# facebookresearch/video-long-term-feature-banks

Hardware: AMD Instinct MI355X
Metric: clips/sec fwd+bwd R50-I3D-NL+LFB-NL, 32x224^2 synthetic (higher is better)
Workload: dtype mix; 1 GPU; ava_r50_lfb_nl fwd+bwd+allreduce+sgd, 8 clips/GPU (global batch 8), RoIs/clip ~ U{1..5} (33 on rank 0), 32x224x224 clips; parallelism=dp1

## Files before the change

video-long-term-feature-banks_amd/csrc/vlfb_gemm_nt.h:

```cpp
#pragma once
#include "vlfb_gemm_common.h"

namespace vlfb {
namespace {

template <typename T, typename OutT, int BM, int BN, bool IDENT, bool DGRAD, bool PACKW, int RB, bool PRE, int NW,
          int ST = 2, bool UT = false, bool PAIR = false, bool W2I = false>
__global__ __launch_bounds__(64 * NW) void gemm_nt_kernel(const GP p) {
  static_assert(!W2I || (sizeof(T) == 2 && RB == 128 && ST == 2 && UT && DGRAD && !PAIR), "W2I: 16-bit unit-stride DGRAD on the tap cursor");
  static_assert(!PAIR || (sizeof(T) == 2 && RB == 128 && ST == 2 && (IDENT || UT) && !PACKW && !DGRAD), "PAIR: fp16 planes, plain rows or UT FPROP");
  static_assert(!UT || (!IDENT && !PACKW), "UT is for gathered, unpacked operands");
  constexpr int NTHR = 64 * NW;
  constexpr int NWN = NW / 2;
  constexpr int EPC = Elem<T>::EPC;
  constexpr int CPRW = RB / 16;
  constexpr int RPPS = NTHR / CPRW;
  constexpr int A_IT = BM / RPPS, B_IT = BN / RPPS;
  constexpr int WM = BM / 2, WN = BN / NWN;
  constexpr int FM = WM / 16, FN = WN / 16;
  constexpr int BUF = (BM + BN) * RB;
  constexpr int KSTEPS = sizeof(T) == 4 ? 1 : RB / 64;
  extern __shared__ __attribute__((aligned(16))) char smem[];

  const int tid = threadIdx.x, lane = tid & 63, wave = tid >> 6;
  const int wm = wave / NWN, wn = wave % NWN;
  const int l15 = lane & 15, g = lane >> 4;

  const int nwg = p.tiles_m * p.tiles_n;
  const int bid = xcd_remap(blockIdx.x, nwg);
  const int tile_m = bid / p.tiles_n, tile_n = bid - tile_m * p.tiles_n;
  int m0 = tile_m * BM;
  const int n0 = tile_n * BN;
  const int z = blockIdx.z;
  constexpr bool S2C = DGRAD && !UT && !IDENT && !PACKW;
  bool s2 = false;
  int s2_ph = 0, s2_pw = 0;
  if constexpr (S2C) {
    s2 = p.s2 != 0;
    if (s2) {
      const int cls = tile_m / p.s2_tpc;
      m0 = (tile_m - cls * p.s2_tpc) * BM;
      s2_ph = cls >> 1; s2_pw = cls & 1;
    }
  }
  const int mrows = s2 ? p.s2_mq : p.M;
  auto row_coords = [&](int m) {
    if constexpr (S2C) {
      if (s2) {
        const int w2n = p.Wr >> 1, h2n = p.Hr >> 1;
        RowC r;
        const int w2 = m % w2n; int q = m / w2n;
        const int h2 = q % h2n; q /= h2n;
        r.t = q % p.Tr; r.n = q / p.Tr;
        r.h = 2 * h2 + s2_ph; r.w = 2 * w2 + s2_pw;
        return r;
      }
    }
    return decode_row(p, m);
  };
  auto row_pos = [&](int m) -> long long {
    if constexpr (S2C) {
      if (s2) {
        const RowC r = row_coords(m);
        return (long long)((r.n * p.Tr + r.t) * p.Hr + r.h) * p.Wr + r.w;
      }
    }
    return m;
  };

  const char* Ab = p.A + (long long)z * p.a_bs * (long long)sizeof(T);
  const char* Bb = p.B + (long long)z * p.b_bs * (long long)sizeof(T);

  const int cc = tid % CPRW;
  const int r0 = tid / CPRW;
  const int ccg = cc ^ swz_key<RB>(r0);
  const unsigned a_cb = PAIR ? (unsigned)(ccg & 3) * 16u + (unsigned)(ccg >> 2) * (unsigned)p.a_ps * 2u : (unsigned)(ccg * EPC) * (unsigned)sizeof(T);
  const unsigned b_cb = PAIR ? (unsigned)(ccg & 3) * 16u + (unsigned)(ccg >> 2) * (unsigned)p.b_ps * 2u : (unsigned)(ccg * EPC) * (unsigned)sizeof(T);
  const int KTB = PAIR ? RB / 2 : RB;
  const int wave_u = __builtin_amdgcn_readfirstlane(wave);

  RowC arow[A_IT];
  bool aok[A_IT];
  int upix[UT ? A_IT : 1];
#pragma unroll
  for (int i = 0; i < A_IT; ++i) {
    int m = m0 + r0 + RPPS * i;
    aok[i] = m < mrows;
    if (!IDENT) arow[i] = row_coords(aok[i] ? m : 0);
    if (UT) {
      RowC& r = arow[i];
      if (!DGRAD) { r.t = r.t * p.st - p.pt; r.h = r.h * p.sh - p.ph; r.w = r.w * p.sw - p.pw; }
      else { r.t += p.pt; r.h += p.ph; r.w += p.pw; }
      upix[i] = ((r.n * p.Ts + r.t) * p.Hs + r.h) * p.Ws + r.w;
    }
  }
  unsigned boff[B_IT], aoff[(IDENT || UT) ? A_IT : 1];
#pragma unroll
  for (int i = 0; i < B_IT; ++i) {
    const int n = n0 + r0 + RPPS * i;
    boff[i] = n < p.Ncols ? (unsigned)(n * p.ldb) * (unsigned)sizeof(T) + b_cb : kOOB;
  }
  if (IDENT || UT) {
#pragma unroll
    for (int i = 0; i < A_IT; ++i) {
      const int m = m0 + r0 + RPPS * i;
      if (IDENT) aoff[i] = aok[i] ? (unsigned)(m * p.lda) * (unsigned)sizeof(T) + a_cb : kOOB;
      else aoff[i] = (unsigned)(upix[i] * p.lda) * (unsigned)sizeof(T) + a_cb;
    }
  }
  const auto rsA = make_rsrc(Ab, p.a_bytes);
  const auto rsB = make_rsrc(Bb, p.b_bytes);
  int u_a = 0, u_b = 0, u_c = 0, u_ci = 0;

  int ktiles = (p.K * (int)sizeof(T) + (PAIR ? RB / 2 : RB) - 1) / (PAIR ? RB / 2 : RB);
  if constexpr (W2I) ktiles *= 2;
  int s2_kpt = 1, s2_b0 = 0, s2_c0 = 0, s2_nb = 0, s2_nc = 0;
  int s2_a = 0, s2_ib = 0, s2_ic = 0, s2_in = 0;
  if constexpr (S2C) {
    if (s2) {
      s2_kpt = p.Cs * (int)sizeof(T) / RB;
      s2_b0 = (s2_ph + p.ph) & 1; s2_c0 = (s2_pw + p.pw) & 1;
      s2_nb = p.kh > s2_b0 ? (p.kh - s2_b0 + 1) >> 1 : 0;
      s2_nc = p.kw > s2_c0 ? (p.kw - s2_c0 + 1) >> 1 : 0;
      ktiles = p.kt * s2_nb * s2_nc * s2_kpt;
    }
  }
  auto s2_next_kt = [&]() {
    const int tap = (s2_a * p.kh + s2_b0 + 2 * s2_ib) * p.kw + s2_c0 + 2 * s2_ic;
    const int kt = tap * s2_kpt + s2_in;
    if (++s2_in == s2_kpt) {
      s2_in = 0;
      if (++s2_ic == s2_nc) { s2_ic = 0; if (++s2_ib == s2_nb) { s2_ib = 0; ++s2_a; } }
    }
    return kt;
  };

  auto load_tile = [&](int kt_seq, int buf) {
    int kt = kt_seq;
    if constexpr (S2C) {
      if (s2) kt = s2_next_kt();
    }
    const int kc = PAIR ? kt * (CPRW / 2) + (ccg & 3) : kt * CPRW + ccg;
    TapC tap;
    if (IDENT || UT) { tap.ok = kc * EPC < p.K; tap.a = tap.b = tap.c = tap.ci = 0; }
    else tap = decode_tap<T, PACKW>(p, kc);
    const bool kok = W2I || kc * EPC < p.K;
    {
      char* xa = smem + (W2I ? (kt_seq >> 1) & 1 : buf) * BUF + wave_u * 1024;
      char* wb = smem + buf * BUF + BM * RB + wave_u * 1024;
      const unsigned kbyte = (unsigned)kt * KTB;
      if (UT) {
        const int sgn = DGRAD ? -1 : 1;
        const int da = sgn * u_a * p.dt, db = sgn * u_b * p.dh, dc = sgn * u_c * p.dw;
        const unsigned dbyte = (unsigned)(((da * p.Hs + db) * p.Ws + dc) * p.lda + u_ci) * (unsigned)sizeof(T);
        if (!W2I || !(kt_seq & 1)) {
#pragma unroll
          for (int i = 0; i < A_IT; ++i) {
            const bool ok = aok[i] && (unsigned)(arow[i].t + da) < (unsigned)p.Ts &&
                            (unsigned)(arow[i].h + db) < (unsigned)p.Hs && (unsigned)(arow[i].w + dc) < (unsigned)p.Ws;
            bufglds16(rsA, ok ? aoff[i] + dbyte : kOOB, 0, xa + i * (RPPS * RB));
          }
          u_ci += (PAIR ? RB / 2 : RB) / (int)sizeof(T);
          if (u_ci >= p.Cs) {
            u_ci = 0;
            if (++u_c == p.kw) { u_c = 0; if (++u_b == p.kh) { u_b = 0; ++u_a; } }
          }
        }
      } else if (IDENT) {
#pragma unroll
        for (int i = 0; i < A_IT; ++i) bufglds16(rsA, kok ? aoff[i] : kOOB, kbyte, xa + i * (RPPS * RB));
      } else {
#pragma unroll
        for (int i = 0; i < A_IT; ++i) {
          unsigned off;
          if (PACKW) {
            const int ts = arow[i].t * p.st - p.pt + tap.a * p.dt;
            const int hs = arow[i].h * p.sh - p.ph + tap.b * p.dh;
            const bool ok = aok[i] && tap.ok && (unsigned)ts < (unsigned)p.Ts && (unsigned)hs < (unsigned)p.Hs;
            const int w0 = arow[i].w * p.sw - p.pw + tap.c;
            const int pix = ((arow[i].n * p.Ts + ts) * p.Hs + hs) * p.Ws + w0;
            off = ok ? (unsigned)pix * 4u * (unsigned)sizeof(T) : kOOB;
          } else {
            bool ok;
            const long long e = src_offset<DGRAD>(p, arow[i], tap, ok);
            off = (ok && aok[i] && tap.ok) ? (unsigned)e * (unsigned)sizeof(T) : kOOB;
          }
          bufglds16(rsA, off, 0, xa + i * (RPPS * RB));
        }
      }
#pragma unroll
      for (int i = 0; i < B_IT; ++i) bufglds16(rsB, kok ? boff[i] : kOOB, kbyte, wb + i * (RPPS * RB));
    }
  };
  constexpr int LPT = A_IT + B_IT;
  auto ring_wait = [&](int newer) {
    if (newer >= 3 && ST >= 5) asm volatile("s_waitcnt vmcnt(%0)" ::"n"(3 * LPT) : "memory");
    else if (newer == 2 && ST >= 4) asm volatile("s_waitcnt vmcnt(%0)" ::"n"(2 * LPT) : "memory");
    else if (newer == 1 && ST >= 3) asm volatile("s_waitcnt vmcnt(%0)" ::"n"(1 * LPT) : "memory");
    else asm volatile("s_waitcnt vmcnt(0)" ::: "memory");
  };

  f32x4_v acc[FN][FM];
#pragma unroll
  for (int a = 0; a < FN; ++a)
#pragma unroll
    for (int b = 0; b < FM; ++b) acc[a][b] = f32x4_v{0.f, 0.f, 0.f, 0.f};

  char* Ob = p.O + (long long)z * p.o_bs * (long long)sizeof(OutT);
  const char* Rb = p.R ? p.R + (long long)z * p.r_bs * (long long)sizeof(T) : nullptr;
  const char* Mb = p.Mask ? p.Mask + (long long)z * p.r_bs * (long long)sizeof(T) : nullptr;
  const char* R2b = p.R2 ? p.R2 + (long long)z * p.r_bs * (long long)sizeof(T) : nullptr;
  char* O2b = p.O2 ? p.O2 + (long long)z * p.o_bs * ((PAIR || sizeof(T) == 2) ? 2ll : (long long)sizeof(OutT)) : nullptr;
  constexpr int EPT = 16 / (int)sizeof(OutT);
  constexpr int TPR = BN / EPT;
  constexpr int RPP = NTHR / TPR;
  constexpr int NPASS = BM / RPP;
  const int tc = tid % TPR, tr = tid / TPR;
  const int ncol = n0 + tc * EPT;
  constexpr bool PREM = PRE && !PAIR;
  constexpr bool PRE2 = PRE && PAIR;
  const bool nt = p.nt_epi != 0;
  uint4 rpre[PRE ? NPASS : 1], mpre[PREM ? NPASS : 1], r2pre[PRE2 ? NPASS : 1];
  if (PRE) {
#pragma unroll
    for (int gp = 0; gp < NPASS; ++gp) {
      const int m = m0 + gp * RPP + tr;
      const bool ok = m < mrows && ncol < p.Ncols;
      const long long off = (row_pos(ok ? m : 0) * p.ldr + ncol) * (long long)sizeof(T);
      rpre[gp] = ld16_epi(nt, src_or_zero(Rb ? Rb : Ab, off, ok && Rb != nullptr));
      if constexpr (PRE2) r2pre[gp] = ld16_epi(nt, src_or_zero(R2b ? R2b : Ab, off, ok && R2b != nullptr));
      if constexpr (PREM) mpre[gp] = ld16_epi(nt, src_or_zero(Mb ? Mb : Ab, off, ok && Mb != nullptr));
    }
  }
  (void)R2b; (void)O2b;

  static_assert(ST >= 2 && ST <= 5 && 3 * LPT < 64, "ring depth / vmcnt immediate");
#pragma unroll
  for (int s0 = 0; s0 < ST - 1; ++s0)
    if (s0 < ktiles) load_tile(s0, s0);

  int cur = 0, nxt = ST - 1;
  if constexpr (W2I) {
    constexpr bool HOLD = !PRE;
    for (int kt = 0; kt < ktiles; kt += 2) {
      typename Mma<T>::Frag xf[KSTEPS][FM];
      asm volatile("s_waitcnt vmcnt(0)" ::: "memory");
      asm volatile("s_barrier" ::: "memory");
      load_tile(kt + 1, 1);
      {
        const char* xa = smem + ((kt >> 1) & 1) * BUF;
        const char* wb = smem + BM * RB;
        if constexpr (HOLD) {
#pragma unroll
          for (int ks = 0; ks < KSTEPS; ++ks)
#pragma unroll
            for (int i = 0; i < FM; ++i) xf[ks][i] = Mma<T>::template load<RB>(xa, wm * WM + i * 16 + l15, ks, g);
        }
#pragma unroll
        for (int ks = 0; ks < KSTEPS; ++ks) {
          typename Mma<T>::Frag wf[FN];
          if constexpr (!HOLD) {
#pragma unroll
            for (int i = 0; i < FM; ++i) xf[ks][i] = Mma<T>::template load<RB>(xa, wm * WM + i * 16 + l15, ks, g);
          }
#pragma unroll
          for (int j = 0; j < FN; ++j) wf[j] = Mma<T>::template load<RB>(wb, wn * WN + j * 16 + l15, ks, g);
#pragma unroll
          for (int j = 0; j < FN; ++j)
#pragma unroll
            for (int i = 0; i < FM; ++i) acc[j][i] = Mma<T>::mma(wf[j], xf[ks][i], acc[j][i]);
        }
      }
      asm volatile("s_waitcnt vmcnt(0)" ::: "memory");
      asm volatile("s_barrier" ::: "memory");
      if (kt + 2 < ktiles) load_tile(kt + 2, 0);
      {
        const char* xa = smem + ((kt >> 1) & 1) * BUF;
        const char* wb = smem + BUF + BM * RB;
#pragma unroll
        for (int ks = 0; ks < KSTEPS; ++ks) {
          typename Mma<T>::Frag wf[FN];
          if constexpr (!HOLD) {
#pragma unroll
            for (int i = 0; i < FM; ++i) xf[ks][i] = Mma<T>::template load<RB>(xa, wm * WM + i * 16 + l15, ks, g);
          }
#pragma unroll
          for (int j = 0; j < FN; ++j) wf[j] = Mma<T>::template load<RB>(wb, wn * WN + j * 16 + l15, ks, g);
#pragma unroll
          for (int j = 0; j < FN; ++j)
#pragma unroll
            for (int i = 0; i < FM; ++i) acc[j][i] = Mma<T>::mma(wf[j], xf[ks][i], acc[j][i]);
        }
      }
    }
  } else
  for (int kt = 0; kt < ktiles; ++kt) {
    const int ahead = ktiles - 1 - kt;
    ring_wait(ahead < ST - 2 ? ahead : ST - 2);
    asm volatile("s_barrier" ::: "memory");
    const bool more = kt + ST - 1 < ktiles;
    if (more) load_tile(kt + ST - 1, nxt);
    const char* xa = smem + cur * BUF;
    const char* wb = xa + BM * RB;
    if constexpr (PAIR) {
      typename Mma<T>::Frag xh[FM], xl[FM], wh[FN], wl[FN];
#pragma unroll
      for (int i = 0; i < FM; ++i) {
        xh[i] = Mma<T>::template load<RB>(xa, wm * WM + i * 16 + l15, 0, g);
        xl[i] = Mma<T>::template load<RB>(xa, wm * WM + i * 16 + l15, 1, g);
      }
#pragma unroll
      for (int j = 0; j < FN; ++j) {
        wh[j] = Mma<T>::template load<RB>(wb, wn * WN + j * 16 + l15, 0, g);
        wl[j] = Mma<T>::template load<RB>(wb, wn * WN + j * 16 + l15, 1, g);
      }
#pragma unroll
      for (int j = 0; j < FN; ++j)
#pragma unroll
        for (int i = 0; i < FM; ++i) acc[j][i] = Mma<T>::mma(wl[j], xh[i], acc[j][i]);
#pragma unroll
      for (int j = 0; j < FN; ++j)
#pragma unroll
        for (int i = 0; i < FM; ++i) acc[j][i] = Mma<T>::mma(wh[j], xl[i], acc[j][i]);
#pragma unroll
      for (int j = 0; j < FN; ++j)
#pragma unroll
        for (int i = 0; i < FM; ++i) acc[j][i] = Mma<T>::mma(wh[j], xh[i], acc[j][i]);
    } else {
#pragma unroll
    for (int ks = 0; ks < KSTEPS; ++ks) {
      typename Mma<T>::Frag xf[FM], wf[FN];
#pragma unroll
      for (int i = 0; i < FM; ++i) xf[i] = Mma<T>::template load<RB>(xa, wm * WM + i * 16 + l15, ks, g);
#pragma unroll
      for (int j = 0; j < FN; ++j) wf[j] = Mma<T>::template load<RB>(wb, wn * WN + j * 16 + l15, ks, g);
#pragma unroll
      for (int j = 0; j < FN; ++j)
#pragma unroll
        for (int i = 0; i < FM; ++i) acc[j][i] = Mma<T>::mma(wf[j], xf[i], acc[j][i]);
    }
    }
    cur = cur + 1 == ST ? 0 : cur + 1;
    nxt = nxt + 1 == ST ? 0 : nxt + 1;
  }
  __syncthreads();

  if (p.vec_epi) {
    constexpr int CPR = BN / 4;
    const int epi = p.epi;
    auto stage = [&](int h) {
      if (epi == 1 || wm == h) {
#pragma unroll
        for (int i = 0; i < FM; ++i) {
          const int row = (epi == 1 ? wm * WM : 0) + i * 16 + l15;
#pragma unroll
          for (int j = 0; j < FN; ++j) {
            const int c = (wn * WN + j * 16 + g * 4) >> 2;
            *reinterpret_cast<float4*>(smem + ((row * CPR + (c ^ (row & 7))) << 4)) =
                make_float4(acc[j][i][0] * p.alpha, acc[j][i][1] * p.alpha, acc[j][i][2] * p.alpha,
                            acc[j][i][3] * p.alpha);
          }
        }
      }
    };
    stage(0);
    __syncthreads();
#pragma unroll
    for (int gp = 0; gp < NPASS; ++gp) {
      if (gp == NPASS / 2 && epi == 2) {
        __syncthreads();
        stage(1);
        __syncthreads();
      }
      const int trow = gp * RPP + tr;
      const int row = (epi == 2 && gp >= NPASS / 2) ? trow - BM / 2 : trow;
      const int m = m0 + trow;
      if (m < mrows && ncol < p.Ncols) {
        const long long mpos = row_pos(m);
        float v[EPT];
#pragma unroll
        for (int q = 0; q < EPT / 4; ++q) {
          const int c = tc * (EPT / 4) + q;
          const float4 t = *reinterpret_cast<const float4*>(smem + ((row * CPR + (c ^ (row & 7))) << 4));
          v[4 * q] = t.x; v[4 * q + 1] = t.y; v[4 * q + 2] = t.z; v[4 * q + 3] = t.w;
        }
        if (p.bias_mode == VLFB_BIAS_COL) {
#pragma unroll
          for (int e = 0; e < EPT; ++e) v[e] += p.bias[ncol + e];
        } else if (p.bias_mode == VLFB_BIAS_ROW) {
          const float b = p.bias[m];
#pragma unroll
          for (int e = 0; e < EPT; ++e) v[e] += b;
        }
        const long long ridx = mpos * p.ldr + ncol;
        if (Rb) {
          float r[EPT];
          if (PRE) unpack_elems<T, EPT>(rpre[PRE ? gp : 0], r);
          else load_elems_epi<T, EPT>(nt, reinterpret_cast<const T*>(Rb) + ridx, r);
#pragma unroll
          for (int e = 0; e < EPT; ++e) v[e] += r[e];
        }
        if constexpr (sizeof(T) == 2 && sizeof(OutT) == 2) {
          if (R2b) {
            float r[EPT];
            if constexpr (PRE2) unpack_elems<T, EPT>(r2pre[PRE2 ? gp : 0], r);
            else load_elems_epi<T, EPT>(nt, reinterpret_cast<const T*>(R2b) + ridx, r);
#pragma unroll
            for (int e = 0; e < EPT; ++e) v[e] += r[e];
          }
        }
        if (p.relu) {
#pragma unroll
          for (int e = 0; e < EPT; ++e) v[e] = fmaxf(v[e], 0.f);
        }
        if (Mb && !PAIR) {
          float r[EPT];
          if (PREM) unpack_elems<T, EPT>(mpre[PREM ? gp : 0], r);
          else load_elems_epi<T, EPT>(nt, reinterpret_cast<const T*>(Mb) + ridx, r);
#pragma unroll
          for (int e = 0; e < EPT; ++e) v[e] = r[e] > 0.f ? v[e] : 0.f;
        }
        OutT* o = reinterpret_cast<OutT*>(Ob) + mpos * p.ldo + ncol;
        if (sizeof(OutT) == 4) {
          st16_epi(nt, o, make_float4(v[0], v[1], v[2], v[3]));
          if constexpr (PAIR) {
            if (O2b) st8_epi(nt, reinterpret_cast<unsigned short*>(O2b) + mpos * p.ldo + ncol,
                             make_uint2(pack_h2_pos(v[0], v[1]), pack_h2_pos(v[2 % EPT], v[3 % EPT])));
          } else if constexpr (sizeof(T) == 2) {
            if (O2b) st8_epi(nt, reinterpret_cast<T*>(O2b) + mpos * p.ldo + ncol,
                             make_uint2(Elem<T>::pack2(v[0], v[1]), Elem<T>::pack2(v[2 % EPT], v[3 % EPT])));
          }
        } else {
          const uint4 hv = make_uint4(Elem<OutT>::pack2(v[0], v[1]), Elem<OutT>::pack2(v[2 % EPT], v[3 % EPT]),
                                      Elem<OutT>::pack2(v[4 % EPT], v[5 % EPT]), Elem<OutT>::pack2(v[6 % EPT], v[7 % EPT]));
          st16_epi(nt, o, hv);
          if (O2b) {
            float h[EPT];
            unpack_elems<OutT, EPT>(hv, h);
            st16_epi(nt, reinterpret_cast<OutT*>(O2b) + mpos * p.ldo + ncol,
                     make_uint4(Elem<OutT>::pack2(v[0] - h[0], v[1] - h[1]), Elem<OutT>::pack2(v[2 % EPT] - h[2 % EPT], v[3 % EPT] - h[3 % EPT]),
                                Elem<OutT>::pack2(v[4 % EPT] - h[4 % EPT], v[5 % EPT] - h[5 % EPT]), Elem<OutT>::pack2(v[6 % EPT] - h[6 % EPT], v[7 % EPT] - h[7 % EPT])));
          }
        }
      }
    }
    return;
  }
  const bool vec_ok = (p.ldo & 3) == 0;
#pragma unroll
  for (int i = 0; i < FM; ++i) {
    const int m = m0 + wm * WM + i * 16 + l15;
    if (m >= mrows) continue;
    const long long mpos = row_pos(m);
#pragma unroll
    for (int j = 0; j < FN; ++j) {
      const int nb = n0 + wn * WN + j * 16 + g * 4;
      if (nb >= p.Ncols) continue;
      const int cnt = (p.Ncols - nb) < 4 ? (p.Ncols - nb) : 4;
      float v[4];
#pragma unroll
      for (int r = 0; r < 4; ++r) {
        float x = acc[j][i][r] * p.alpha;
        if (r < cnt) {
          if (p.bias_mode == VLFB_BIAS_COL) x += p.bias[nb + r];
          else if (p.bias_mode == VLFB_BIAS_ROW) x += p.bias[m];
          if (Rb) x += ld_elem<T>(Rb, mpos * p.ldr + nb + r);
          if (p.relu) x = fmaxf(x, 0.f);
          if (Mb) x = ld_elem<T>(Mb, mpos * p.ldr + nb + r) > 0.f ? x : 0.f;
        }
        v[r] = x;
      }
      store4<OutT>(Ob, mpos * p.ldo + nb, v, cnt, vec_ok);
    }
  }
}

}
}
```

video-long-term-feature-banks_amd/csrc/vlfb_gemm_pair.hip:

```cpp
#include "vlfb_gemm_nt.h"
#include "vlfb_gemm_nt8.h"

namespace vlfb {
namespace {

template <typename K>
void launch_pair_k(K kernel, dim3 grid, int threads, size_t lds, const GP& gp, hipStream_t s) {
  static bool configured = false;
  if (!configured) {
    (void)hipFuncSetAttribute(reinterpret_cast<const void*>(kernel), hipFuncAttributeMaxDynamicSharedMemorySize, 80 * 1024);
    configured = true;
  }
  hipLaunchKernelGGL(kernel, grid, dim3(threads), lds, s, gp);
}

template <typename OutT, int BN, bool PRE>
void launch_pair_shape(const GP& gp, bool ident, dim3 grid, size_t lds, hipStream_t s) {
  constexpr int NW = 8;
  if (ident) launch_pair_k(gemm_nt_kernel<f16_t, OutT, 128, BN, true, false, false, 128, PRE, NW, 2, false, true>, grid, 64 * NW, lds, gp, s);
  else launch_pair_k(gemm_nt_kernel<f16_t, OutT, 128, BN, false, false, false, 128, PRE, NW, 2, true, true>, grid, 64 * NW, lds, gp, s);
}

template <auto Kernel>
void launch_pair8_k(const GP& gp, dim3 grid, size_t lds, hipStream_t s) {
  static bool configured = false;
  if (!configured) {
    (void)hipFuncSetAttribute(reinterpret_cast<const void*>(Kernel), hipFuncAttributeMaxDynamicSharedMemorySize, 160 * 1024);
    configured = true;
  }
  hipLaunchKernelGGL(Kernel, grid, dim3(512), lds, s, gp);
}
template <typename OutT, int BN, int RV>
void launch_pair8_bn(const GP& gp, int mode, dim3 grid, hipStream_t s) {
  constexpr size_t lds = (BN == 256 ? 2 : 3) * (size_t)(2 + BN / 128) * 16384;
  if (mode == 0) launch_pair8_k<gemm_nt8_kernel<f16_t, OutT, BN, 0, false, RV, true>>(gp, grid, lds, s);
  else launch_pair8_k<gemm_nt8_kernel<f16_t, OutT, BN, 1, false, RV, true>>(gp, grid, lds, s);
}
template <typename OutT>
void launch_pair8_t(const GP& gp, int mode, int bm, int bn, dim3 grid, hipStream_t s) {
  if (bn == 256) {
    if (bm == 196) launch_pair8_bn<OutT, 256, 98>(gp, mode, grid, s); else launch_pair8_bn<OutT, 256, 128>(gp, mode, grid, s);
  } else {
    if (bm == 196) launch_pair8_bn<OutT, 128, 98>(gp, mode, grid, s); else launch_pair8_bn<OutT, 128, 128>(gp, mode, grid, s);
  }
}

}

int launch_nt8_pair(const GP& gp, int bm, int bn, int mode, bool out_f32, hipStream_t s) {
  const dim3 grid((unsigned)(gp.tiles_m * gp.tiles_n), 1, 1);
  if (out_f32) launch_pair8_t<float>(gp, mode, bm, bn, grid, s); else launch_pair8_t<f16_t>(gp, mode, bm, bn, grid, s);
  return check_launch("conv kernel (fp16 planes, 256-row pipelined)");
}

int launch_nt_pair(const GP& gp, int bn, bool ident, bool pre, bool out_f32, dim3 grid, size_t lds, hipStream_t s) {
  if (out_f32) {
    if (bn == 64) launch_pair_shape<float, 64, false>(gp, ident, grid, lds, s);
    else launch_pair_shape<float, 128, false>(gp, ident, grid, lds, s);
  } else if (pre) {
    if (bn == 64) launch_pair_shape<f16_t, 64, true>(gp, ident, grid, lds, s);
    else launch_pair_shape<f16_t, 128, true>(gp, ident, grid, lds, s);
  } else {
    if (bn == 64) launch_pair_shape<f16_t, 64, false>(gp, ident, grid, lds, s);
    else launch_pair_shape<f16_t, 128, false>(gp, ident, grid, lds, s);
  }
  return check_launch("conv kernel (fp16 planes)");
}

}
```

Measured before the change: 263.7 clips/s.

## Make fp16 pair GEMM persistent, prefetching the next tile's K-loop during the epilogue

Adds a LOOP variant of the pair GEMM kernel that launches about two workgroups per CU and has each walk over several output tiles. On the last k-step of a tile it stages the next tile's row offsets and issues the first load, then runs the epilogue through the other LDS slot, so the epilogue overlaps the next tile's loads. By default this applies to identity-row (1x1) pair GEMMs whose tile count exceeds the slot count. In exchange it adds register pressure from the waves-per-EU hint and the extra state, forces epi=2 staging, and risks load imbalance when tiles don't divide evenly across slots.

```diff
diff --git a/video-long-term-feature-banks_amd/csrc/vlfb_gemm_nt.h b/video-long-term-feature-banks_amd/csrc/vlfb_gemm_nt.h
--- a/video-long-term-feature-banks_amd/csrc/vlfb_gemm_nt.h
+++ b/video-long-term-feature-banks_amd/csrc/vlfb_gemm_nt.h
@@ -5,8 +5,9 @@
 namespace {
 
 template <typename T, typename OutT, int BM, int BN, bool IDENT, bool DGRAD, bool PACKW, int RB, bool PRE, int NW,
-          int ST = 2, bool UT = false, bool PAIR = false, bool W2I = false>
-__global__ __launch_bounds__(64 * NW) void gemm_nt_kernel(const GP p) {
+          int ST = 2, bool UT = false, bool PAIR = false, bool W2I = false, bool LOOP = false>
+__global__ __launch_bounds__(64 * NW) __attribute__((amdgpu_waves_per_eu(LOOP ? 4 : 1))) void gemm_nt_kernel(const GP p) {
+  static_assert(!LOOP || (PAIR && ST == 2 && (BM / 2) * BN * 4 <= (BM + BN) * RB), "LOOP: two-plane instances, two slots, half a tile per slot");
   static_assert(!W2I || (sizeof(T) == 2 && RB == 128 && ST == 2 && UT && DGRAD && !PAIR), "W2I: 16-bit unit-stride DGRAD on the tap cursor");
   static_assert(!PAIR || (sizeof(T) == 2 && RB == 128 && ST == 2 && (IDENT || UT) && !PACKW && !DGRAD), "PAIR: fp16 planes, plain rows or UT FPROP");
   static_assert(!UT || (!IDENT && !PACKW), "UT is for gathered, unpacked operands");
@@ -27,10 +28,11 @@
   const int l15 = lane & 15, g = lane >> 4;
 
   const int nwg = p.tiles_m * p.tiles_n;
-  const int bid = xcd_remap(blockIdx.x, nwg);
+  int wg = blockIdx.x;
+  const int bid = xcd_remap(wg, nwg);
   const int tile_m = bid / p.tiles_n, tile_n = bid - tile_m * p.tiles_n;
   int m0 = tile_m * BM;
-  const int n0 = tile_n * BN;
+  int n0 = tile_n * BN;
   const int z = blockIdx.z;
   constexpr bool S2C = DGRAD && !UT && !IDENT && !PACKW;
   bool s2 = false;
@@ -82,6 +84,8 @@
   RowC arow[A_IT];
   bool aok[A_IT];
   int upix[UT ? A_IT : 1];
+  unsigned boff[B_IT], aoff[(IDENT || UT) ? A_IT : 1];
+  auto stage_rows = [&]() {
 #pragma unroll
   for (int i = 0; i < A_IT; ++i) {
     int m = m0 + r0 + RPPS * i;
@@ -94,7 +98,6 @@
       upix[i] = ((r.n * p.Ts + r.t) * p.Hs + r.h) * p.Ws + r.w;
     }
   }
-  unsigned boff[B_IT], aoff[(IDENT || UT) ? A_IT : 1];
 #pragma unroll
   for (int i = 0; i < B_IT; ++i) {
     const int n = n0 + r0 + RPPS * i;
@@ -108,6 +111,8 @@
       else aoff[i] = (unsigned)(upix[i] * p.lda) * (unsigned)sizeof(T) + a_cb;
     }
   }
+  };
+  stage_rows();
   const auto rsA = make_rsrc(Ab, p.a_bytes);
   const auto rsB = make_rsrc(Bb, p.b_bytes);
   int u_a = 0, u_b = 0, u_c = 0, u_ci = 0;
@@ -200,12 +205,6 @@
     else asm volatile("s_waitcnt vmcnt(0)" ::: "memory");
   };
 
-  f32x4_v acc[FN][FM];
-#pragma unroll
-  for (int a = 0; a < FN; ++a)
-#pragma unroll
-    for (int b = 0; b < FM; ++b) acc[a][b] = f32x4_v{0.f, 0.f, 0.f, 0.f};
-
   char* Ob = p.O + (long long)z * p.o_bs * (long long)sizeof(OutT);
   const char* Rb = p.R ? p.R + (long long)z * p.r_bs * (long long)sizeof(T) : nullptr;
   const char* Mb = p.Mask ? p.Mask + (long long)z * p.r_bs * (long long)sizeof(T) : nullptr;
@@ -216,12 +215,12 @@
   constexpr int RPP = NTHR / TPR;
   constexpr int NPASS = BM / RPP;
   const int tc = tid % TPR, tr = tid / TPR;
-  const int ncol = n0 + tc * EPT;
   constexpr bool PREM = PRE && !PAIR;
   constexpr bool PRE2 = PRE && PAIR;
   const bool nt = p.nt_epi != 0;
   uint4 rpre[PRE ? NPASS : 1], mpre[PREM ? NPASS : 1], r2pre[PRE2 ? NPASS : 1];
-  if (PRE) {
+  auto pre_rows = [&]() {
+    const int ncol = n0 + tc * EPT;
 #pragma unroll
     for (int gp = 0; gp < NPASS; ++gp) {
       const int m = m0 + gp * RPP + tr;
@@ -231,7 +230,8 @@
       if constexpr (PRE2) r2pre[gp] = ld16_epi(nt, src_or_zero(R2b ? R2b : Ab, off, ok && R2b != nullptr));
       if constexpr (PREM) mpre[gp] = ld16_epi(nt, src_or_zero(Mb ? Mb : Ab, off, ok && Mb != nullptr));
     }
-  }
+  };
+  if (PRE) pre_rows();
   (void)R2b; (void)O2b;
 
   static_assert(ST >= 2 && ST <= 5 && 3 * LPT < 64, "ring depth / vmcnt immediate");
@@ -240,6 +240,14 @@
     if (s0 < ktiles) load_tile(s0, s0);
 
   int cur = 0, nxt = ST - 1;
+  for (;;) {
+  const int em0 = m0, en0 = n0, ncol = n0 + tc * EPT;
+  const bool walk = LOOP && wg + (int)gridDim.x < nwg;
+  f32x4_v acc[FN][FM];
+#pragma unroll
+  for (int a = 0; a < FN; ++a)
+#pragma unroll
+    for (int b = 0; b < FM; ++b) acc[a][b] = f32x4_v{0.f, 0.f, 0.f, 0.f};
   if constexpr (W2I) {
     constexpr bool HOLD = !PRE;
     for (int kt = 0; kt < ktiles; kt += 2) {
@@ -300,6 +308,17 @@
     asm volatile("s_barrier" ::: "memory");
     const bool more = kt + ST - 1 < ktiles;
     if (more) load_tile(kt + ST - 1, nxt);
+    if constexpr (LOOP) {
+      if (!more && walk) {
+        wg += (int)gridDim.x;
+        const int nb = xcd_remap(wg, nwg);
+        const int tm = nb / p.tiles_n;
+        m0 = tm * BM; n0 = (nb - tm * p.tiles_n) * BN;
+        stage_rows();
+        u_a = u_b = u_c = u_ci = 0;
+        load_tile(0, nxt);
+      }
+    }
     const char* xa = smem + cur * BUF;
     const char* wb = xa + BM * RB;
     if constexpr (PAIR) {
@@ -348,6 +367,7 @@
   if (p.vec_epi) {
     constexpr int CPR = BN / 4;
     const int epi = p.epi;
+    char* const stg = LOOP ? smem + nxt * BUF : smem;
     auto stage = [&](int h) {
       if (epi == 1 || wm == h) {
 #pragma unroll
@@ -356,7 +376,7 @@
 #pragma unroll
           for (int j = 0; j < FN; ++j) {
             const int c = (wn * WN + j * 16 + g * 4) >> 2;
-            *reinterpret_cast<float4*>(smem + ((row * CPR + (c ^ (row & 7))) << 4)) =
+            *reinterpret_cast<float4*>(stg + ((row * CPR + (c ^ (row & 7))) << 4)) =
                 make_float4(acc[j][i][0] * p.alpha, acc[j][i][1] * p.alpha, acc[j][i][2] * p.alpha,
                             acc[j][i][3] * p.alpha);
           }
@@ -374,14 +394,14 @@
       }
       const int trow = gp * RPP + tr;
       const int row = (epi == 2 && gp >= NPASS / 2) ? trow - BM / 2 : trow;
-      const int m = m0 + trow;
+      const int m = em0 + trow;
       if (m < mrows && ncol < p.Ncols) {
         const long long mpos = row_pos(m);
         float v[EPT];
 #pragma unroll
         for (int q = 0; q < EPT / 4; ++q) {
           const int c = tc * (EPT / 4) + q;
-          const float4 t = *reinterpret_cast<const float4*>(smem + ((row * CPR + (c ^ (row & 7))) << 4));
+          const float4 t = *reinterpret_cast<const float4*>(stg + ((row * CPR + (c ^ (row & 7))) << 4));
           v[4 * q] = t.x; v[4 * q + 1] = t.y; v[4 * q + 2] = t.z; v[4 * q + 3] = t.w;
         }
         if (p.bias_mode == VLFB_BIAS_COL) {
@@ -444,17 +464,19 @@
         }
       }
     }
-    return;
+    if (!walk) return;
+    if (PRE) pre_rows();
+    continue;
   }
   const bool vec_ok = (p.ldo & 3) == 0;
 #pragma unroll
   for (int i = 0; i < FM; ++i) {
-    const int m = m0 + wm * WM + i * 16 + l15;
+    const int m = em0 + wm * WM + i * 16 + l15;
     if (m >= mrows) continue;
     const long long mpos = row_pos(m);
 #pragma unroll
     for (int j = 0; j < FN; ++j) {
-      const int nb = n0 + wn * WN + j * 16 + g * 4;
+      const int nb = en0 + wn * WN + j * 16 + g * 4;
       if (nb >= p.Ncols) continue;
       const int cnt = (p.Ncols - nb) < 4 ? (p.Ncols - nb) : 4;
       float v[4];
@@ -473,6 +495,9 @@
       store4<OutT>(Ob, mpos * p.ldo + nb, v, cnt, vec_ok);
     }
   }
+  if (!walk) return;
+  if (PRE) pre_rows();
+  }
 }
 
 }
diff --git a/video-long-term-feature-banks_amd/csrc/vlfb_gemm_pair.hip b/video-long-term-feature-banks_amd/csrc/vlfb_gemm_pair.hip
--- a/video-long-term-feature-banks_amd/csrc/vlfb_gemm_pair.hip
+++ b/video-long-term-feature-banks_amd/csrc/vlfb_gemm_pair.hip
@@ -14,9 +14,44 @@
   hipLaunchKernelGGL(kernel, grid, dim3(threads), lds, s, gp);
 }
 
+int loop_slots() {
+  static int slots = 0;
+  if (!slots) {
+    int dev = 0, cus = 0;
+    if (hipGetDevice(&dev) != hipSuccess || hipDeviceGetAttribute(&cus, hipDeviceAttributeMultiprocessorCount, dev) != hipSuccess || cus <= 0) {
+      (void)hipGetLastError();
+      return 0;
+    }
+    slots = (2 * cus + 7) / 8 * 8;
+  }
+  return slots;
+}
+unsigned loop_grid(const GP& gp, bool ident, dim3 grid) {
+  static const int mode = env_int("VLFB_NT_TILE_LOOP", 1);
+  static const int cap = env_int("VLFB_NT_LOOP_WGS", 0);
+  if (mode <= 0 || !gp.vec_epi || grid.y != 1) return 0;
+  const int tiles = gp.tiles_m * gp.tiles_n;
+  if ((int)grid.x != tiles) return 0;
+  int slots = loop_slots();
+  if (cap > 0 && cap < slots) slots = cap;
+  if (slots <= 0) return 0;
+  if (mode >= 2) return (unsigned)(tiles < slots ? tiles : slots);
+  if (!ident || tiles <= slots) return 0;
+  return (unsigned)slots;
+}
+
 template <typename OutT, int BN, bool PRE>
 void launch_pair_shape(const GP& gp, bool ident, dim3 grid, size_t lds, hipStream_t s) {
   constexpr int NW = 8;
+  if (const unsigned lg = loop_grid(gp, ident, grid)) {
+    GP lp = gp;
+    lp.epi = 2;
+    const dim3 lgrid(lg, 1, grid.z);
+    const size_t llds = (size_t)2 * (128 + BN) * 128;
+    if (ident) launch_pair_k(gemm_nt_kernel<f16_t, OutT, 128, BN, true, false, false, 128, PRE, NW, 2, false, true, false, true>, lgrid, 64 * NW, llds, lp, s);
+    else launch_pair_k(gemm_nt_kernel<f16_t, OutT, 128, BN, false, false, false, 128, PRE, NW, 2, true, true, false, true>, lgrid, 64 * NW, llds, lp, s);
+    return;
+  }
   if (ident) launch_pair_k(gemm_nt_kernel<f16_t, OutT, 128, BN, true, false, false, 128, PRE, NW, 2, false, true>, grid, 64 * NW, lds, gp, s);
   else launch_pair_k(gemm_nt_kernel<f16_t, OutT, 128, BN, false, false, false, 128, PRE, NW, 2, true, true>, grid, 64 * NW, lds, gp, s);
 }
```

New measurement: 260.1 clips/s. -1.4%, worse.
